# LANL-Bioinformatics/PCRamp

Hardware: AMD Instinct MI355X
Metric: primer-pair x target amplification evals/sec (higher is better)
Workload: dtype u32

## Files before the change

pcramp_amd/csrc/pcr_device.hip:

```cpp
#include <hip/hip_runtime.h>
#include <cstring>
#include <rocprim/device/device_radix_sort.hpp>

#include <stdint.h>
#include <string.h>
#include <math.h>
#include <stdlib.h>
#include <string>
#include <vector>
#include <chrono>
#include <algorithm>
#include <unordered_map>
#include <type_traits>
#include <thread>
#include <mutex>
#include <condition_variable>
#include <functional>
#include <memory>

#include "../../include/pcramp_hip.h"
#include "pcr_host.hpp"

using pcrhost::Planes;

// ... 152 lines not shown
	const uint32_t tagged = (k.epoch << 8) | cnt;
	const uint32_t old = atomicMax(&k.best[(size_t)seq*k.ncand + cand], tagged);
	if(tagged >= old){
		const uint32_t slot = atomicAdd(&k.seq_count[seq], 1u);
		if(slot < k.cap){
			Hit h; h.key = key; h.cand = cand; h.cnt = cnt;
			k.hits[(size_t)seq*k.cap + slot] = h;
		}
		else{ atomicOr(&k.counters[0], 1u); atomicMax(&k.counters[2], slot + 1); }
	}
}

__device__ __noinline__ void record_hit(const HitSink k, uint32_t seq, uint32_t cand, uint64_t key, uint32_t cnt)
{
	record_hit_inline(k, seq, cand, key, cnt);
}

__device__ __forceinline__ uint64_t make_key(uint32_t seq, int32_t loc, uint32_t strand , uint32_t kind, uint32_t ord)
{
	return ((uint64_t)seq << KEY_SEQ_SHIFT) | ((uint64_t)(uint32_t)(loc + LOC_BIAS) << KEY_LOC_SHIFT) |
		((uint64_t)(strand - 1) << 7) | ((uint64_t)kind << 6) | ord;
}

__global__ void k_touched(const uint32_t *__restrict__ seq_count, uint32_t n, uint32_t *__restrict__ counters, uint32_t *__restrict__ touched)
{
	const uint32_t s = blockIdx.x*blockDim.x + threadIdx.x;
	const uint32_t fill = (s < n) ? seq_count[s] : 0u;
	const bool has = fill > 0;
	const uint64_t mask = __ballot(has);
	if(!mask) return;
// ... 426 lines not shown
	pcrhost::PackFilter filt;
	SeqSet sets[PCR_N_SETS];
	DevBuf<uint32_t> best, counters, mask, status;
	int scan_version = 3;
	bool force_seed1 = false;
	std::vector<uint32_t> s2_seeds; std::vector<uint4> s2_masks; std::vector<uint8_t> s2_floors;
	std::vector<uint32_t> s2_group_end, s2_group_offmask, s2_group_or, s2_group_nor;
	struct S2Key { uint32_t a, c, g, t, floor_; bool operator==(const S2Key &o) const { return a == o.a && c == o.c && g == o.g && t == o.t && floor_ == o.floor_; } };
	struct S2KeyHash { size_t operator()(const S2Key &k) const { uint64_t h = 0x9E3779B97F4A7C15ull; for(uint32_t v : {k.a, k.c, k.g, k.t, k.floor_}){ h ^= v; h *= 0x100000001B3ull; h ^= h >> 29; } return (size_t)h; } };
	struct S2Entry { std::vector<uint32_t> seeds;  uint32_t off_mask; bool seedable; uint4 mask;
		std::vector<uint32_t> chunks; uint32_t chunks_total = 0; uint64_t chunks_gen = 0;  };
	std::unordered_map<S2Key, S2Entry, S2KeyHash> s2_cache;
	std::vector<pcrhost::Seed> s2_tmp;
	struct S3Launch { Seed3Slices W; uint32_t n_chunks, per_wg, slice_cap, n_irr_wg; };
	std::vector<S3Launch> s3_launch;
	std::vector<uint32_t> s3_prefix; bool no_seed3 = false, s3_attr_set = false;
	bool s2_attr_set = false; uint32_t s2_dbg = 0; bool no_irr_index = false;
	std::vector<uint32_t> s1_seeds; std::unordered_map<S2Key, S2Entry, S2KeyHash> s1_cache;
	DevBuf<uint32_t> s1_image, s1_heads, s1_multi, s1_part;
	bool host_seed_tables = false;
	DevBuf<Hit> hits;
	DevBuf<uint64_t> bits_fr, bits_rf;
	DevBuf<OligoDev> oligos;
	DevBuf<SwJob> sw_jobs; DevBuf<SwOut> sw_out; DevBuf<uint8_t> sw_q, sw_qlen, sw_t, entry_codes, entry_lens;
	DevBuf<AmpRec> amp_recs, amp_recs2; DevBuf<BgPairDev> bg_pairs;
	DevBuf<uint64_t> amp_keys; DevBuf<uint32_t> amp_pkeys, amp_pair_start; DevBuf<uint8_t> sort_tmp;
	DevBuf<thermo::Job> th_jobs; DevBuf<thermo::JobOut> th_out; DevBuf<int> th_dg; DevBuf<uint2> th_map; DevBuf<uint32_t> th_bad;
	float th_dg_salt = -1.0f;
	DevBuf<unsigned long long> th_dbg; bool th_attr_set = false;
	std::vector<thermo::Job> th_host_jobs; std::vector<thermo::JobOut> th_host_res;
// ... 715 lines not shown
	}
	memset((void *)ctx->mail, 0, sizeof(pcr_ctx::Mail)*pcr_ctx::MAIL_RING);
	return ctx;
}

void pcr_destroy(pcr_ctx *ctx)
{
	if(!ctx) return;
	(void)hipSetDevice(ctx->device);
	(void)hipStreamSynchronize(ctx->stream);
	ctx->pending.clear();
	if(ctx->timing && ctx->n_timed){
		const double n = (double)ctx->n_timed;
		fprintf(stderr, "[pcramp] host us/pass: plan %.1f  stage %.1f  launch %.1f  wait %.1f | amplify prep %.1f  launch %.1f  (%llu passes)\n",
			ctx->t_host[0]/n, ctx->t_host[1]/n, ctx->t_host[2]/n, ctx->t_host[3]/n, ctx->t_host[4]/n, ctx->t_host[5]/n, (unsigned long long)ctx->n_timed);
	}
	for(auto &pr : ctx->prof_events){ (void)hipEventDestroy(pr.first); (void)hipEventDestroy(pr.second); }
	for(int k = 0;k < PCR_PROF_KERNELS;++k){ for(auto &pr : ctx->prof_events_k[k]){ (void)hipEventDestroy(pr.first); (void)hipEventDestroy(pr.second); } }
	for(int s = 0;s < PCR_N_SETS;++s) ctx->sets[s].release();
	ctx->best.release();
	ctx->counters.release(); ctx->mask.release(); ctx->status.release(); ctx->hits.release();
	ctx->s1_image.release(); ctx->s1_heads.release(); ctx->s1_multi.release(); ctx->s1_part.release();
	ctx->bits_fr.release(); ctx->bits_rf.release(); ctx->arena.release(); ctx->fin_scratch.release();
	for(auto &sl : ctx->stage){ if(sl.host) (void)hipHostFree(sl.host); if(sl.done) (void)hipEventDestroy(sl.done); }
	for(auto &sl : ctx->dstage){ if(sl.dev) (void)hipFree(sl.dev); }
	if(ctx->mail) (void)hipHostFree(ctx->mail);
	if(ctx->ret_host) (void)hipHostFree(ctx->ret_host);
	if(ctx->in_host) (void)hipHostFree(ctx->in_host);
	if(ctx->ret_flag) (void)hipHostFree(ctx->ret_flag);
	if(ctx->sw_pin) (void)hipHostFree(ctx->sw_pin);
	for(int k = 0;k < 2;++k){ if(ctx->sw_done[k]) (void)hipEventDestroy(ctx->sw_done[k]); }
// ... 241 lines not shown
	return pcr_split_many(ctx, which, &seq, &pos, 1);
}

}

namespace {

inline uint32_t spread16(uint32_t v)
{
	v &= 0xFFFFu;
	v = (v | (v << 8)) & 0x00FF00FFu; v = (v | (v << 4)) & 0x0F0F0F0Fu;
	v = (v | (v << 2)) & 0x33333333u; return (v | (v << 1)) & 0x55555555u;
}

constexpr uint32_t S2_MAX_GROUPS = 4096;
bool plan_seed2(pcr_ctx *ctx, const std::vector<pcrhost::Candidate> &cand, std::vector<uint32_t> &or_seed, std::vector<uint32_t> &or_plain, uint32_t &irr_off_mask,
	const SeqSet *S3 = nullptr)
{
	std::vector<uint32_t> &pf = ctx->s3_prefix;
	pf.clear();
	uint32_t pf_run = 0;
	const uint32_t n_or = 2*(uint32_t)cand.size();
	std::vector<uint32_t> &out = ctx->s2_seeds;
	out.clear(); ctx->s2_group_end.clear(); ctx->s2_group_offmask.clear(); ctx->s2_group_or.clear(); ctx->s2_group_nor.clear();
	irr_off_mask = 0;
	ctx->s2_masks.resize(n_or);
	if(ctx->s2_cache.size() > 16384) ctx->s2_cache.clear();
	size_t group_begin = 0; uint32_t group_mask = 0, group_or0 = 0, group_last = 0;
	auto fits = [&](size_t n, uint32_t g_or){
		if(S3) return g_or <= S3_MAX_OR && n <= S3_MAX_SEEDS;
		return g_or <= S2_MAX_OR && n <= S2_MAX_SEEDS && sizeof(S2Shared) + 17*(size_t)g_or + 8*n + 1024 <= 160*1024;
	};
	for(uint32_t o = 0;o < n_or;++o){
		const pcrhost::Candidate &c = cand[o >> 1];
		const Planes &m = (o & 1u) ? c.rc : c.fwd;
		const pcr_ctx::S2Key key = {m.a, m.c, m.g, m.t, c.floor_};
		auto it = ctx->s2_cache.find(key);
		if(it == ctx->s2_cache.end()){
			pcr_ctx::S2Entry e; e.off_mask = 0;
			ctx->s2_tmp.clear();
			e.seedable = pcrhost::orientation_seeds(m, c.floor_, 0, ctx->s2_tmp, nullptr, S2_Q);
			e.mask = make_uint4(spread16(m.a) | (spread16(m.a >> 16) << 1), spread16(m.c) | (spread16(m.c >> 16) << 1),
			                    spread16(m.g) | (spread16(m.g >> 16) << 1), spread16(m.t) | (spread16(m.t >> 16) << 1));
			e.seeds.reserve(ctx->s2_tmp.size());
			for(const pcrhost::Seed &sd : ctx->s2_tmp){ e.seeds.push_back((sd.code << 14) | ((uint32_t)sd.off << 9)); e.off_mask |= 1u << sd.off; }
			it = ctx->s2_cache.emplace(key, std::move(e)).first;
		}
		pcr_ctx::S2Entry &e = it->second;
		ctx->s2_masks[o] = e.mask;
		if(!e.seedable){ or_plain.push_back(o); continue; }
		or_seed.push_back(o);
		if(!fits(out.size() - group_begin + e.seeds.size(), o - group_or0 + 1)){
			if(!fits(e.seeds.size(), 1) || ctx->s2_group_end.size() + 1 >= S2_MAX_GROUPS) return false;
			ctx->s2_group_end.push_back((uint32_t)out.size()); ctx->s2_group_offmask.push_back(group_mask); ctx->s2_group_or.push_back(group_or0); ctx->s2_group_nor.push_back(group_last - group_or0 + 1);
			group_begin = out.size(); group_mask = 0; group_or0 = o;
			if(S3){ pf.push_back(pf_run); pf_run = 0; }
		}
		group_last = o;
		const size_t at = out.size();
		out.resize(at + e.seeds.size());
		for(size_t k = 0;k < e.seeds.size();++k) out[at + k] = e.seeds[k] | (o - group_or0);
		if(S3){
			if(e.chunks_gen != S3->pix_generation){
				e.chunks.resize(e.seeds.size());
				uint32_t run = 0;
				for(size_t k = 0;k < e.seeds.size();++k){ e.chunks[k] = run; run += (S3->pix_count_h[e.seeds[k] >> 14] + 63u) >> 6; }
				e.chunks_total = run; e.chunks_gen = S3->pix_generation;
			}
			const size_t pa = pf.size();
			pf.resize(pa + e.chunks.size());
			for(size_t k = 0;k < e.chunks.size();++k) pf[pa + k] = pf_run + e.chunks[k];
			pf_run += e.chunks_total;
		}
		if(!(o & 1u)){ irr_off_mask |= e.off_mask; group_mask |= e.off_mask; }
	}
	ctx->s2_group_end.push_back((uint32_t)out.size()); ctx->s2_group_offmask.push_back(group_mask); ctx->s2_group_or.push_back(group_or0);
	ctx->s2_group_nor.push_back(or_seed.empty() ? 0u : group_last - group_or0 + 1);
	if(S3) pf.push_back(pf_run);
	return true;
}

constexpr size_t S3_LDS_BUDGET = 120*1024;
uint32_t seed3_grid(const pcr_ctx *ctx, int *wg_threads)
{
	static const int s3_wg = getenv("PCRAMP_S3_WG") ? atoi(getenv("PCRAMP_S3_WG")) : 1024;
	static const int s3_per_cu = getenv("PCRAMP_S3_PER_CU") ? atoi(getenv("PCRAMP_S3_PER_CU")) : 0;
	if(wg_threads) *wg_threads = (s3_wg == 1024) ? 1024 : 512;
	return std::min<uint32_t>(ctx->n_cu*(uint32_t)(s3_per_cu ? s3_per_cu : (s3_wg == 1024 ? 2 : 4)), S3_MAX_WG);
}
bool plan_seed3_slices(pcr_ctx *ctx, bool with_irr)
{
	int wg_threads = 0;
	const uint32_t G_all = seed3_grid(ctx, &wg_threads);
	ctx->s3_launch.resize(ctx->s2_group_end.size());
	size_t g_begin = 0, g_prefix = 0;
	for(size_t g = 0;g < ctx->s2_group_end.size();++g){
		const uint32_t ns = ctx->s2_group_end[g] - (uint32_t)g_begin;
		g_begin = ctx->s2_group_end[g];
		const uint32_t *P = ctx->s3_prefix.data() + g_prefix;
		g_prefix += (size_t)ns + 1;
		pcr_ctx::S3Launch &L = ctx->s3_launch[g];
		L.n_irr_wg = with_irr ? std::min<uint32_t>((ns + 16u*(uint32_t)(wg_threads/64) - 1u)/(16u*(uint32_t)(wg_threads/64)), G_all/4u) : 0u;
		const uint32_t G = G_all - L.n_irr_wg;
		L.n_chunks = P[ns]; L.per_wg = std::max<uint32_t>(1u, (L.n_chunks + G - 1u)/G); L.slice_cap = 2;
		if(ns == 0) continue;
		uint32_t at = 0;
		for(uint32_t w = 0;w <= G;++w){
			const uint64_t target = (uint64_t)w*L.per_wg;
			while(at + 1u < ns && P[at + 1u] <= target) ++at;
			L.W.start[w] = at;
		}
		for(uint32_t w = G + 1;w <= S3_MAX_WG;++w) L.W.start[w] = at;
		for(uint32_t w = 0;w < G;++w) L.slice_cap = std::max(L.slice_cap, std::min(L.W.start[w + 1] + 2u, ns + 1u) - L.W.start[w]);
		if(17*(size_t)ctx->s2_group_nor[g] + 8*(size_t)L.slice_cap + 64 > S3_LDS_BUDGET) return false;
	}
	return true;
}

void plan_seed1(pcr_ctx *ctx, const std::vector<pcrhost::Candidate> &cand, std::vector<uint32_t> &or_seed, std::vector<uint32_t> &or_plain, uint32_t &irr_off_mask)
{
	const uint32_t n_or = 2*(uint32_t)cand.size();
	std::vector<uint32_t> &out = ctx->s1_seeds;
	out.clear();
	irr_off_mask = 0;
	if(ctx->s1_cache.size() > 16384) ctx->s1_cache.clear();
// ... 177 lines not shown

int select_impl(pcr_ctx *ctx, pcr_set which, const pcr_pair *pairs, uint32_t n_pairs, int optimize_5, int optimize_3,
	float threshold, uint32_t min_oligo_length, uint64_t *n_entries_out, bool async, FusedAmp *fa = nullptr)
{
	if(!ctx || (n_pairs && !pairs)){ g_err = "pcr_select_words: bad argument"; return PCR_ERR_ARG; }
	if(min_oligo_length < 1 || min_oligo_length > 32){ g_err = "pcr_select_words: min_oligo_length must be in [1,32]"; return PCR_ERR_ARG; }
	HIP_TRY(hipSetDevice(ctx->device));
	SeqSet &S = ctx->sets[which];
	S.have_db = false; S.n_entries = 0;
	if(n_entries_out) *n_entries_out = 0;
	const bool ctrl_was_clean = S.ctrl_clean;
	S.ctrl_clean = false; S.touched_from_seg = false;
	bool lean = false, cleared_bits = false; size_t lean_bits_bytes = 0;
	HostTimer timer(ctx, 0);
	if(ctx->timing) ++ctx->n_timed;
	std::vector<pcrhost::Candidate> cand;
	pcrhost::build_candidates((const uint64_t *)pairs, n_pairs, optimize_5 != 0, optimize_3 != 0, threshold, cand);
	const uint32_t ncand = (uint32_t)cand.size();
	if(S.n == 0 || ncand == 0){ S.have_db = true; S.n_touched = 0; return PCR_OK; }
	std::vector<uint4> hf(ncand), hr(ncand); std::vector<uint32_t> hfl(ncand);
	for(uint32_t c = 0;c < ncand;++c){
		hf[c] = make_uint4(cand[c].fwd.a, cand[c].fwd.c, cand[c].fwd.g, cand[c].fwd.t);
		hr[c] = make_uint4(cand[c].rc.a, cand[c].rc.c, cand[c].rc.g, cand[c].rc.t);
		hfl[c] = cand[c].floor_;
	}
	int rc;
	if((rc = ctx->best.ensure((size_t)S.n*ncand)) != PCR_OK) return rc;
	if(ctx->best.generation != ctx->best_seen){
		HIP_TRY(hipMemsetAsync(ctx->best.p, 0, ctx->best.cap*sizeof(uint32_t), ctx->stream));
		ctx->best_seen = ctx->best.generation; ctx->epoch = std::min(ctx->debug_epoch, EPOCH_LIMIT);
	}
	const uint32_t n_or = 2*ncand;
	std::vector<uint32_t> or_seed, or_plain;
	HostSeedPlan H;
	uint32_t irr_off_mask = 0;
	bool want_seed3 = false, s3_with_irr = false;
	if(ctx->scan_version == 3 && !ctx->force_seed1 && !optimize_5 && !optimize_3 && n_or <= 65535 && !ctx->no_seed3 && !ctx->no_irr_index && ctx->s2_dbg == 0){
		bool worth = true;
		if(!S.pix_valid){
			std::vector<uint32_t> os, op; uint32_t om = 0;
			worth = plan_seed2(ctx, cand, os, op, om, nullptr) && op.empty() && !os.empty();
		}
		if(worth){
			int irc = ensure_pos_index(ctx, S);
			if(irc != PCR_OK) return irc;
			uint32_t n_live0 = 0;
			for(uint32_t k = std::min<uint32_t>(min_oligo_length, 256);k < 256;++k) n_live0 += S.irr_size_count[k];
			bool irr_ok = n_live0 == 0;
			if(S.pix_usable && !irr_ok && S.irr_n_multi == 0 && (uint64_t)24*S.n_irr < (uint64_t(1) << 32)){
				if((irc = ensure_irr_index(ctx, S)) != PCR_OK) return irc;
				irr_ok = S.irx_usable;
			}
			want_seed3 = S.pix_usable && irr_ok; s3_with_irr = n_live0 > 0;
		}
	}
	bool use_seed2 = false;
	if(ctx->scan_version == 3 && !ctx->force_seed1 && !optimize_5 && !optimize_3 && n_or <= 65535){
		use_seed2 = plan_seed2(ctx, cand, or_seed, or_plain, irr_off_mask, want_seed3 ? &S : nullptr);
		if(want_seed3 && !(use_seed2 && or_plain.empty() && !or_seed.empty() && plan_seed3_slices(ctx, s3_with_irr))){
			or_seed.clear(); or_plain.clear();
			use_seed2 = plan_seed2(ctx, cand, or_seed, or_plain, irr_off_mask, nullptr);
		}
		if(use_seed2 && !or_plain.empty() && (n_or <= S1_MAX_OR || or_seed.empty())) use_seed2 = false;
		if(!use_seed2){ or_seed.clear(); or_plain.clear(); irr_off_mask = 0; }
	}
	const bool use_seed3 = use_seed2 && want_seed3 && or_plain.empty() && !or_seed.empty()
		&& ctx->s3_prefix.size() == ctx->s2_seeds.size() + ctx->s2_group_end.size();
	bool dev_tables = false;
	if(!use_seed2 && ctx->scan_version == 3 && !ctx->host_seed_tables && !optimize_5 && !optimize_3 && n_or <= S1_MAX_OR){
		plan_seed1(ctx, cand, or_seed, or_plain, irr_off_mask);
		dev_tables = true;
	}
	if(use_seed2 || dev_tables){  }
	else if(ctx->scan_version == 3 && n_or <= 65535){
// ... 17 lines not shown
	const uint32_t *d_tab_seedset = nullptr, *d_bias_seedset = nullptr, *d_map_seedset = nullptr;
	{
		size_t bytes = ncand*(2*sizeof(uint4) + sizeof(uint32_t)) + 1024;
		bytes += (tab_plain.tab.size() + tab_plain.bias.size() + or_plain.size() + 256)*sizeof(uint32_t);
		bytes += (tab_seedset.tab.size() + tab_seedset.bias.size() + or_seed.size() + 256)*sizeof(uint32_t);
		bytes += (H.image.size() + H.heads.size() + H.multi.size() + 64)*sizeof(uint32_t);
		std::vector<uint4> &masks2 = ctx->s2_masks; std::vector<uint8_t> &floors2 = ctx->s2_floors;
		if(use_seed2){
			floors2.assign(((size_t)n_or + 15) & ~size_t(15), 0);
			for(uint32_t o = 0;o < n_or;++o) floors2[o] = (uint8_t)std::min<uint32_t>(cand[o >> 1].floor_, 255u);
			bytes += masks2.size()*sizeof(uint4) + floors2.size() + ctx->s2_seeds.size()*sizeof(uint32_t) + 512;
			if(use_seed3) bytes += ctx->s3_prefix.size()*sizeof(uint32_t) + 64;
		}
		const bool build_tables = dev_tables && !or_seed.empty();
		if(build_tables) bytes += ctx->s1_seeds.size()*sizeof(uint32_t) + 256;
		std::vector<OligoDev> ol;
		size_t bits_bytes = 0;
		bool fuse = false;
		if(fa && fa->n_pairs){
			bits_bytes = (size_t)fa->n_pairs*((S.n + 63)/64)*sizeof(uint64_t);
			fuse = ((uintptr_t)fa->d_fr % 16 == 0) && ((uintptr_t)fa->d_rf % 16 == 0) && (bits_bytes % 16 == 0);
			if(fuse){ build_oligos(fa->pairs, fa->n_pairs, fa->a, ol); bytes += ol.size()*sizeof(OligoDev) + 64; }
		}
		timer.next(1);
		{
			const uint64_t gen = S.ctrl.generation;
			if((rc = S.ctrl.ensure(8 + 2*(size_t)S.n + 4)) != PCR_OK) return rc;
			lean = ctx->direct_ok && async && fuse && use_seed2 && !or_seed.empty() && ctrl_was_clean && gen == S.ctrl.generation
				&& S.bucket_cap == POST_CAP && 2*fa->n_pairs <= 32*POST_MASK_WORDS;
			lean_bits_bytes = bits_bytes;
		}
// ... 130 lines not shown
						}
						if(use_seed3){
							Seed3Tables T3; T3.seeds = Tg.seeds; T3.chunk_prefix = d_s3_prefix + g_prefix; T3.masks = Tg.masks; T3.floors = Tg.floors;
							g_prefix += Tg.n_seeds + 1u;
							T3.n_seeds = Tg.n_seeds; T3.n_or = Tg.n_or; T3.or_base = Tg.or_base;
							T3.pix_first = S.pix_first.p; T3.pix_last = S.pix_last.p; T3.pix_ent = S.pix_ent.p;
							Seed3Set Q3 = { S.valid_d(), S.blk_info.p, S.blk_local.p, S.d_active.p };
							int s3_wg = 0;
							const uint32_t G = seed3_grid(ctx, &s3_wg);
							const pcr_ctx::S3Launch &L3 = ctx->s3_launch[g];
							T3.n_chunks = L3.n_chunks; T3.per_wg = L3.per_wg; T3.slice_cap = L3.slice_cap;
							T3.n_irr_wg = IA.ix_first ? L3.n_irr_wg : 0u;
							const Seed3Slices &W3 = L3.W;
							const size_t dyn3 = (size_t)g_or*sizeof(uint4) + 2*(size_t)T3.slice_cap*sizeof(uint32_t) + (((size_t)g_or + 15) & ~size_t(15)) + 16;
							if(!ctx->s3_attr_set){
								HIP_TRY(hipFuncSetAttribute((const void *)k_seed3<512>, hipFuncAttributeMaxDynamicSharedMemorySize, 128*1024));
								HIP_TRY(hipFuncSetAttribute((const void *)k_seed3<1024>, hipFuncAttributeMaxDynamicSharedMemorySize, 128*1024));
								ctx->s3_attr_set = true;
							}
							if(s3_wg == 1024) hipLaunchKernelGGL(k_seed3<1024>, dim3(G), dim3(1024), dyn3, ctx->stream, T3, Q3, IA, ctx->d_cand_fwd, ctx->d_cand_floor, sink, Z, W3);
							else hipLaunchKernelGGL(k_seed3<512>, dim3(G), dim3(512), dyn3, ctx->stream, T3, Q3, IA, ctx->d_cand_fwd, ctx->d_cand_floor, sink, Z, W3);
						}
						else if(ctx->s2_dbg)
							hipLaunchKernelGGL(k_seed2<true>, sgrid, sblock, dyn, ctx->stream, S.tb_d(), S.valid_d(), S.tile_desc.p, S.n_tiles, Tg, S.d_active.p, ctx->d_cand_fwd, ctx->d_cand_floor, ncand, IA, sink,
							ctx->s2_dbg, Z);
						else
							hipLaunchKernelGGL(k_seed2<false>, sgrid, sblock, dyn, ctx->stream, S.tb_d(), S.valid_d(), S.tile_desc.p, S.n_tiles, Tg, S.d_active.p, ctx->d_cand_fwd, ctx->d_cand_floor, ncand, IA, sink,
							ctx->s2_dbg, Z);
						HIP_TRY(hipGetLastError());
						first_launch = false;
					}
					if(need_seedset && (rc = launch_scan2(ctx, S, tab_seedset, ncand, sink, d_tab_seedset, d_bias_seedset, S.degen_tiles.p,
						S.n_degen_tiles, d_map_seedset)) != PCR_OK) return rc;
				}
				else if(!or_seed.empty()){
					const bool cand_lds = ncand <= SEED_CAND_LDS;
// ... 458 lines not shown
```

pcramp_amd/csrc/pcr_scan_seed3.inc:

```

constexpr uint32_t PIX_CODES = 1u << 18;
constexpr uint32_t S3_BATCH = 8;

template<bool SCATTER>
__global__ void k_pix_build(const uint32_t *__restrict__ tb, const uint32_t *__restrict__ blk_seq, const uint64_t *__restrict__ blk_off,
	const uint64_t *__restrict__ len, uint64_t total_blocks, uint32_t *__restrict__ count_or_cursor, uint4 *__restrict__ ent)
{
	const uint64_t b = (uint64_t)blockIdx.x*blockDim.x + threadIdx.x;
	if(b >= total_blocks) return;
	const uint32_t seq = blk_seq[b];
	const int64_t p0 = (int64_t)(b - blk_off[seq])*32, L = (int64_t)len[seq];
	uint32_t w[8];
#pragma unroll
	for(int k = 0;k < 8;++k) w[k] = tb[(int64_t)2*(int64_t)b - 2 + k];
#pragma unroll
	for(int i = 0;i < 32;++i){
		if(p0 + i + 9 > L) break;
		const uint32_t code = ((i < 16) ? funnel(w[2], w[3], 2*i) : funnel(w[3], w[4], 2*(i - 16))) & S2_CODE_MASK;
		if(SCATTER){
			const uint32_t at = atomicAdd(&count_or_cursor[code], 1u);
			const int jl = (i + 9) >> 4, sl = 2*((i + 9) & 15);
			const int jr = (i + 41) >> 4, sr = 2*((i + 41) & 15);
			const uint32_t l_lo = funnel(w[jl], w[jl + 1], sl), l_hi = funnel(w[jl + 1], w[jl + 2], sl) & 0x3FFFu;
			const uint32_t r_lo = funnel(w[jr], w[jr + 1], sr), r_hi = funnel(w[jr + 1], w[jr + 2], sr) & 0x3FFFu;
// ... 30 lines not shown
	const uint64_t bl = b - blk_off[q], tile = bl >> 5;
	const uint32_t nt = tile0[q + 1] - tile0[q];
	const bool degen = tile < nt && tile_degen[tile0[q] + tile];
	blk_info[b] = q | (degen ? 0x80000000u : 0u) | (active[q] ? 0u : 0x40000000u);
	blk_local[b] = (uint32_t)bl;
}

__global__ void k_blk_active(uint32_t *__restrict__ blk_info, const uint32_t *__restrict__ blk_seq, const uint8_t *__restrict__ active, uint64_t total_blocks)
{
	const uint64_t b = (uint64_t)blockIdx.x*blockDim.x + threadIdx.x;
	if(b >= total_blocks) return;
	const uint32_t v = blk_info[b] & ~BLK_INACTIVE;
	blk_info[b] = v | (active[blk_seq[b]] ? 0u : BLK_INACTIVE);
}

__device__ __forceinline__ void s3_irregular(const Seed3Tables &T3, const Seed3Set &Q, const IrrArgs2 &IA, const uint4 *__restrict__ cand_fwd,
	const uint32_t *__restrict__ cand_floor, HitSink sink, uint32_t gw, uint32_t n_gw, uint32_t lane)
{
	for(uint32_t i0 = gw*16u;i0 < T3.n_seeds;i0 += n_gw*16u){
		const uint32_t i = i0 + lane;
		const uint32_t sdv = (lane < 16u && i < T3.n_seeds) ? T3.seeds[i] : S2_END;
		const uint32_t orient = T3.or_base + (sdv & 0x1FFu);
		uint32_t first = 0, cnt = 0;
		if(sdv != S2_END && !(orient & 1u)){
			const uint32_t key = (((sdv >> 9) & 31u) << 18) | (sdv >> 14);
			first = IA.ix_first[key]; cnt = IA.ix_last[key] - first;
		}
		const uint32_t incl = s2_scan(cnt);
		const uint32_t total = s2_rl(incl, 63);
		for(uint32_t t0 = 0;t0 < total;t0 += 64u){
			const uint32_t t = t0 + lane;
			uint32_t lo = 0;
#pragma unroll
			for(uint32_t stp = 32u;stp;stp >>= 1){ if((uint32_t)__shfl((int)incl, (int)(lo + stp - 1u)) <= t) lo += stp; }
			const int sl = (int)min(lo, 63u);
			const uint32_t s_incl = (uint32_t)__shfl((int)incl, sl), s_cnt = (uint32_t)__shfl((int)cnt, sl), s_first = (uint32_t)__shfl((int)first, sl);
			const uint32_t c = (uint32_t)__shfl((int)orient, sl) >> 1;
			if(t >= total) continue;
			const IrrDev e = IA.irr[IA.ix_words[s_first + (t - (s_incl - s_cnt))]];
			if(((e.meta >> 8) & 0xFFu) < IA.min_cws || !Q.active[e.seq]) continue;
			const uint32_t n = match_count(e.w.a, e.w.c, e.w.g, e.w.t, cand_fwd[c]);
			if(n >= cand_floor[c]) record_hit(sink, e.seq, c, make_key(e.seq, e.loc, e.meta & 0xFF, 1, (e.meta >> 16) & 0xFF), n);
		}
	}
}

template<uint32_t S3_THREADS>
__global__ __launch_bounds__(S3_THREADS) __attribute__((amdgpu_waves_per_eu(8, 8))) void k_seed3(Seed3Tables T3, Seed3Set Q, IrrArgs2 IA, const uint4 *__restrict__ cand_fwd, const uint32_t *__restrict__ cand_floor,
	HitSink sink, S2Clear Z, Seed3Slices W)
{
	extern __shared__ uint4 s3_dyn[];
	uint4 *const masks = s3_dyn;
	uint32_t *const prefix = (uint32_t *)(masks + T3.n_or);
	uint32_t *const seeds = prefix + T3.slice_cap;
	uint8_t *const floors = (uint8_t *)(seeds + T3.slice_cap);
	const uint32_t wave = threadIdx.x >> 6, lane = threadIdx.x & 63u;
	for(uint32_t i = blockIdx.x*S3_THREADS + threadIdx.x;i < Z.n0;i += gridDim.x*S3_THREADS) Z.z0[i] = make_uint4(0, 0, 0, 0);
	for(uint32_t i = blockIdx.x*S3_THREADS + threadIdx.x;i < Z.n1;i += gridDim.x*S3_THREADS) Z.z1[i] = make_uint4(0, 0, 0, 0);
	if(Z.ctrl && blockIdx.x == 0 && threadIdx.x == 0){ Z.ctrl[1] = 0; Z.ctrl[3] = 0; }
	for(uint32_t i = threadIdx.x;i < T3.n_or;i += S3_THREADS){ masks[i] = T3.masks[i]; floors[i] = T3.floors[i]; }
	constexpr uint32_t S3_WAVES = S3_THREADS/64;
	if(blockIdx.x < T3.n_irr_wg){
		if(IA.ix_first) s3_irregular(T3, Q, IA, cand_fwd, cand_floor, sink, blockIdx.x*S3_WAVES + wave, T3.n_irr_wg*S3_WAVES, lane);
		return;
	}
	const uint32_t wg = blockIdx.x - T3.n_irr_wg, n_wg = gridDim.x - T3.n_irr_wg;
	const uint32_t s_lo = W.start[wg];
	const uint32_t n_slice = min(min(W.start[wg + 1] + 2u, T3.n_seeds + 1u) - s_lo, T3.slice_cap);
	for(uint32_t i = threadIdx.x;i < n_slice;i += S3_THREADS){ prefix[i] = T3.chunk_prefix[s_lo + i]; seeds[i] = (s_lo + i < T3.n_seeds) ? T3.seeds[s_lo + i] : 0u; }
	__syncthreads();
	const uint32_t gw = wg*S3_WAVES + wave, n_gw = n_wg*S3_WAVES;
	const uint32_t q_lo = wg*T3.per_wg, q_hi = min(q_lo + T3.per_wg, T3.n_chunks);
	for(uint32_t q0 = q_lo + wave;q0 < q_hi;q0 += S3_WAVES*S3_BATCH){
		uint32_t c_first = 0, c_cnt = 0, c_sd = 0;
		{
			const uint32_t q = q0 + lane*S3_WAVES;
			if(lane < S3_BATCH && q < q_hi){
				uint32_t lo = 0, hi = n_slice - 1u;
// ... 30 lines not shown
		for(int b = 0;b < (int)S3_BATCH;++b){
			vw[b] = 0; info[b] = 0; bl[b] = 0;
			if(pass_b[b]){
				const uint32_t ws = g[b] - ((s2_rl(c_sd, b) >> 9) & 31u);
				vw[b] = Q.valid[ws >> 5]; info[b] = Q.blk_info[ws >> 5]; bl[b] = Q.blk_local[ws >> 5];
			}
		}
#pragma unroll
		for(int b = 0;b < (int)S3_BATCH;++b){
			if(!pass_b[b]) continue;
			const uint32_t sdv = s2_rl(c_sd, b);
			const uint32_t ws = g[b] - ((sdv >> 9) & 31u), seq = info[b] & BLK_SEQ_MASK;
			if(!((vw[b] >> (ws & 31u)) & 1u) || (info[b] & (BLK_DEGEN | BLK_INACTIVE))) continue;
			const uint32_t p_local = bl[b]*32u + (ws & 31u);
			const uint32_t orient = T3.or_base + (sdv & 0x1FFu), c = orient >> 1;
			if(orient & 1u) record_hit(sink, seq, c, make_key(seq, (int32_t)p_local + 31, 2, 0, 0), cnt_b[b]);
			else record_hit(sink, seq, c, make_key(seq, (int32_t)p_local, 1, 0, 0), cnt_b[b]);
		}
	}
	if(IA.ix_first && T3.n_irr_wg == 0) s3_irregular(T3, Q, IA, cand_fwd, cand_floor, sink, gw, n_gw, lane);
}
```

pcramp_amd/csrc/pcr_screen.inc:

```
__device__ __forceinline__ bool db_slot(uint32_t g, uint32_t n, uint32_t cap, const uint32_t *__restrict__ touched,
	const uint32_t *__restrict__ seg_hi, uint32_t &slot)
{
	if(g >= n) return false;
	const uint32_t seq = touched[g/cap];
	slot = seq*cap + g % cap;
	return slot < seg_hi[seq];
}

constexpr int MATCH_WAVES = 4;
__global__ __launch_bounds__(64*MATCH_WAVES) void k_match(const DevEntry *__restrict__ db, uint32_t n_touched, const uint32_t *__restrict__ n_touched_dev, uint32_t cap,
	const uint32_t *__restrict__ touched, const uint32_t *__restrict__ seg_hi, const OligoDev *__restrict__ oligos, uint32_t n_oligo,
	uint32_t mask_words, uint32_t *__restrict__ mask, uint32_t *__restrict__ status,
	const uint32_t *__restrict__ pub_counters, PassMail *pub_mail, uint32_t pub_seq)
{
	if(blockIdx.x == 0 && threadIdx.x == 0 && status) status[0] = 0;
	if(pub_mail && blockIdx.x == 0 && threadIdx.x < 64){
		if(threadIdx.x < 4) pub_mail->counters[threadIdx.x] = pub_counters[threadIdx.x];
		__threadfence_system();
		__builtin_amdgcn_wave_barrier();
		if(threadIdx.x == 0) __hip_atomic_store((uint32_t *)&pub_mail->seq, pub_seq, __ATOMIC_RELEASE, __HIP_MEMORY_SCOPE_SYSTEM);
	}
	if(n_touched_dev) n_touched = *n_touched_dev;
	const uint32_t lane = threadIdx.x & 63u, sub = lane >> 5, ol = lane & 31u;
	for(uint32_t t_idx = blockIdx.x*MATCH_WAVES + (threadIdx.x >> 6);t_idx < n_touched;t_idx += gridDim.x*MATCH_WAVES){
// ... 262 lines not shown
			const float f = (side == 0) ? var : best, r2 = (side == 0) ? best : var;
			if(__fsqrt_rn(__fmul_rn(f, r2)) >= ident_thr)
				atomicOr((unsigned long long *)&dst[(size_t)v*bit_words + (seq >> 6)], bit);
		}
	}
}

constexpr uint32_t POST_CAP = 64, POST_MASK_WORDS = 4;
struct PostEnt { Planes w; int32_t loc; uint32_t strand; };
template<int POST_WAVES>
struct PostShared {
	OligoDev ol[32*POST_MASK_WORDS];
	uint64_t keys[POST_WAVES][POST_CAP]; PostEnt ent[POST_WAVES][POST_CAP]; uint32_t msk[POST_WAVES][POST_CAP][POST_MASK_WORDS];
};

template<int POST_WAVES>
__global__ __launch_bounds__(64*POST_WAVES) void k_post(const Hit *__restrict__ hits, uint32_t *__restrict__ seq_count,
	const uint32_t *__restrict__ best, uint32_t ncand, const uint4 *__restrict__ planes, const uint64_t *__restrict__ blk_off,
	const IrrDev *__restrict__ irr, const uint32_t *__restrict__ irr_off, DevEntry *__restrict__ db, uint32_t *__restrict__ seg_hi,
	uint32_t *__restrict__ counters, uint32_t epoch, uint32_t n_seq,
	const OligoDev *__restrict__ oligos, uint32_t n_pairs, uint32_t mask_words,
	const uint64_t *__restrict__ len, const uint8_t *__restrict__ active, int32_t amp_min, int32_t amp_max, float ident_thr, int use_taq,
	uint64_t *__restrict__ bits_fr, uint64_t *__restrict__ bits_rf, uint64_t bit_words, PassMail *pub_mail, uint32_t pub_seq)
{
	__shared__ PostShared<POST_WAVES> sh;
	const uint32_t wave = threadIdx.x >> 6, lane = threadIdx.x & 63u;
	if(pub_mail && blockIdx.x == 0 && wave == 0){
		if(lane < 4) pub_mail->counters[lane] = (lane == 3) ? N_TOUCHED_UNKNOWN_DEV : counters[lane];
		__threadfence_system();
		__builtin_amdgcn_wave_barrier();
		if(lane == 0) __hip_atomic_store((uint32_t *)&pub_mail->seq, pub_seq, __ATOMIC_RELEASE, __HIP_MEMORY_SCOPE_SYSTEM);
	}
	if(blockIdx.x == 0 && wave == 0 && lane < 4) counters[lane] = 0;
	const uint32_t seq = blockIdx.x*POST_WAVES + wave;
	const uint32_t n_raw = (seq < n_seq) ? seq_count[seq] : 0u;
	const uint32_t n = min(n_raw, POST_CAP);
	if(seq < n_seq && lane == 0){
		if(n_raw) seq_count[seq] = 0;
		else seg_hi[seq] = 0;
	}
	const uint32_t seq_c = min(seq, n_seq - 1u);
	const uint64_t base = blk_off[seq_c];
	const int32_t L = (int32_t)len[seq_c];
	const uint32_t is_active = active[seq_c];
	if(__syncthreads_or((int)n)){
		const uint32_t nw = 2*n_pairs*(uint32_t)(sizeof(OligoDev)/4);
		for(uint32_t i = threadIdx.x;i < nw;i += 64*POST_WAVES) ((uint32_t *)sh.ol)[i] = ((const uint32_t *)oligos)[i];
		__syncthreads();
	}
	if(n == 0) return;
	uint64_t *keys = sh.keys[wave];
	PostEnt *ent = sh.ent[wave];
	uint64_t k = ~0ull;
	if(lane < n){
		const Hit h = hits[(size_t)seq*POST_CAP + lane];
		if(((epoch << 8) | h.cnt) == best[(size_t)seq*ncand + h.cand]) k = h.key;
	}
	keys[lane] = k;
	wave_sync();
	uint32_t np2 = 1; while(np2 < n) np2 <<= 1;
	for(uint32_t kk = 2;kk <= np2;kk <<= 1){
		for(uint32_t j = kk >> 1;j > 0;j >>= 1){
			const uint32_t l = lane ^ j;
			if(l > lane && l < np2){
				const uint64_t a = keys[lane], b = keys[l];
				const bool up = ((lane & kk) == 0);
				if((a > b) == up){ keys[lane] = b; keys[l] = a; }
			}
			wave_sync();
		}
	}
	k = keys[lane];
// ... 215 lines not shown
```

Before: 19.76 billion.

## Append seed3 hits without atomicMax and resolve per-candidate best in k_post

Adds an APPEND variant of k_seed3 that writes hits straight into the per-sequence list, skipping the global atomicMax on the best table. k_post now computes each candidate's maximum count itself by scanning the wave's hits in LDS. The variant is used in lean mode. On the host, the seed3 workgroup slice boundaries are computed during the plan_seed2 prefix walk rather than in a second pass, and per-pass vectors are reused from the context. Without the atomicMax filter, more hits may reach the per-sequence cap and overflow. The k_post scan is O(n) per lane over at most 64 entries.

After: 20.53 billion (median of 6 runs). 1.04x the previous value.

```diff
diff --git a/pcramp_amd/csrc/pcr_device.hip b/pcramp_amd/csrc/pcr_device.hip
--- a/pcramp_amd/csrc/pcr_device.hip
+++ b/pcramp_amd/csrc/pcr_device.hip
@@ -190,6 +190,23 @@
 __device__ __noinline__ void record_hit(const HitSink k, uint32_t seq, uint32_t cand, uint64_t key, uint32_t cnt)
 {
 	record_hit_inline(k, seq, cand, key, cnt);
+}
+
+__device__ __noinline__ void append_hit(const HitSink k, uint32_t seq, uint32_t cand, uint64_t key, uint32_t cnt)
+{
+	const uint32_t slot = atomicAdd(&k.seq_count[seq], 1u);
+	if(slot < k.cap){
+		Hit h; h.key = key; h.cand = cand; h.cnt = cnt;
+		k.hits[(size_t)seq*k.cap + slot] = h;
+	}
+	else{ atomicOr(&k.counters[0], 1u); atomicMax(&k.counters[2], slot + 1); }
+}
+
+template<bool APPEND>
+__device__ __forceinline__ void sink_hit(const HitSink &k, uint32_t seq, uint32_t cand, uint64_t key, uint32_t cnt)
+{
+	if(APPEND) append_hit(k, seq, cand, key, cnt);
+	else record_hit(k, seq, cand, key, cnt);
 }
 
 __device__ __forceinline__ uint64_t make_key(uint32_t seq, int32_t loc, uint32_t strand , uint32_t kind, uint32_t ord)
@@ -646,6 +663,9 @@
 	std::vector<pcrhost::Seed> s2_tmp;
 	struct S3Launch { Seed3Slices W; uint32_t n_chunks, per_wg, slice_cap, n_irr_wg; };
 	std::vector<S3Launch> s3_launch;
+	std::vector<S2Entry *> s2_ent;
+	bool s3_walked = false; uint32_t s3_walk_G = 0, s3_walk_per_wg = 0;
+	std::vector<pcrhost::Candidate> pass_cand; std::vector<uint4> pass_hf, pass_hr; std::vector<uint32_t> pass_hfl; std::vector<OligoDev> pass_ol;
 	std::vector<uint32_t> s3_prefix; bool no_seed3 = false, s3_attr_set = false;
 	bool s2_attr_set = false; uint32_t s2_dbg = 0; bool no_irr_index = false;
 	std::vector<uint32_t> s1_seeds; std::unordered_map<S2Key, S2Entry, S2KeyHash> s1_cache;
@@ -1391,7 +1411,19 @@
 		const double n = (double)ctx->n_timed;
 		fprintf(stderr, "[pcramp] host us/pass: plan %.1f  stage %.1f  launch %.1f  wait %.1f | amplify prep %.1f  launch %.1f  (%llu passes)\n",
 			ctx->t_host[0]/n, ctx->t_host[1]/n, ctx->t_host[2]/n, ctx->t_host[3]/n, ctx->t_host[4]/n, ctx->t_host[5]/n, (unsigned long long)ctx->n_timed);
-	}
+		fprintf(stderr, "[pcramp] host: of the plan, workgroup slices %.1f us/pass; index builds (once per set, not in the plan) %.1f ms\n",
+			ctx->t_host[7]/n, ctx->t_host[6]*1e-3);
+	}
+#ifdef PCRAMP_FILL_HIST
+	{
+		uint32_t h[257];
+		if(hipMemcpyFromSymbol(h, HIP_SYMBOL(g_fill_hist), sizeof(h)) == hipSuccess){
+			fprintf(stderr, "[pcramp] bucket fills offered to k_post (fill:sequence-passes):");
+			for(int i = 0;i < 257;++i) if(h[i]) fprintf(stderr, " %d:%u", i, h[i]);
+			fprintf(stderr, "\n");
+		}
+	}
+#endif
 	for(auto &pr : ctx->prof_events){ (void)hipEventDestroy(pr.first); (void)hipEventDestroy(pr.second); }
 	for(int k = 0;k < PCR_PROF_KERNELS;++k){ for(auto &pr : ctx->prof_events_k[k]){ (void)hipEventDestroy(pr.first); (void)hipEventDestroy(pr.second); } }
 	for(int s = 0;s < PCR_N_SETS;++s) ctx->sets[s].release();
@@ -1663,9 +1695,12 @@
 }
 
 constexpr uint32_t S2_MAX_GROUPS = 4096;
+uint32_t seed3_grid(const pcr_ctx *ctx, int *wg_threads);
+uint32_t s3_irr_wgs(uint32_t ns, int wg_threads, uint32_t G_all, bool with_irr);
 bool plan_seed2(pcr_ctx *ctx, const std::vector<pcrhost::Candidate> &cand, std::vector<uint32_t> &or_seed, std::vector<uint32_t> &or_plain, uint32_t &irr_off_mask,
-	const SeqSet *S3 = nullptr)
-{
+	const SeqSet *S3 = nullptr, bool s3_with_irr = false)
+{
+	ctx->s3_walked = false;
 	std::vector<uint32_t> &pf = ctx->s3_prefix;
 	pf.clear();
 	uint32_t pf_run = 0;
@@ -1680,6 +1715,9 @@
 		if(S3) return g_or <= S3_MAX_OR && n <= S3_MAX_SEEDS;
 		return g_or <= S2_MAX_OR && n <= S2_MAX_SEEDS && sizeof(S2Shared) + 17*(size_t)g_or + 8*n + 1024 <= 160*1024;
 	};
+	std::vector<pcr_ctx::S2Entry *> &ent = ctx->s2_ent;
+	ent.resize(n_or);
+	size_t tot_seeds = 0; uint64_t tot_chunks = 0; uint32_t o_first = n_or, o_last = 0;
 	for(uint32_t o = 0;o < n_or;++o){
 		const pcrhost::Candidate &c = cand[o >> 1];
 		const Planes &m = (o & 1u) ? c.rc : c.fwd;
@@ -1696,6 +1734,30 @@
 			it = ctx->s2_cache.emplace(key, std::move(e)).first;
 		}
 		pcr_ctx::S2Entry &e = it->second;
+		ent[o] = &e;
+		if(!e.seedable) continue;
+		if(S3 && e.chunks_gen != S3->pix_generation){
+			e.chunks.resize(e.seeds.size());
+			uint32_t run = 0;
+			for(size_t k = 0;k < e.seeds.size();++k){ e.chunks[k] = run; run += (S3->pix_count_h[e.seeds[k] >> 14] + 63u) >> 6; }
+			e.chunks_total = run; e.chunks_gen = S3->pix_generation;
+		}
+		tot_seeds += e.seeds.size(); tot_chunks += S3 ? e.chunks_total : 0u;
+		o_first = std::min(o_first, o); o_last = o;
+	}
+	pcr_ctx::S3Launch *WL = nullptr;
+	uint32_t w_next = 0, w_G = 0, w_per = 0; uint64_t w_target = 0;
+	if(S3 && tot_seeds && fits(tot_seeds, o_last - o_first + 1) && tot_chunks < (uint64_t(1) << 32)){
+		int wg_threads = 0;
+		const uint32_t G_all = seed3_grid(ctx, &wg_threads);
+		w_G = G_all - s3_irr_wgs((uint32_t)tot_seeds, wg_threads, G_all, s3_with_irr);
+		w_per = std::max<uint32_t>(1u, (uint32_t)((tot_chunks + w_G - 1u)/w_G));
+		ctx->s3_launch.resize(1);
+		WL = &ctx->s3_launch[0];
+		WL->W.start[0] = 0; w_next = 1; w_target = w_per;
+	}
+	for(uint32_t o = 0;o < n_or;++o){
+		pcr_ctx::S2Entry &e = *ent[o];
 		ctx->s2_masks[o] = e.mask;
 		if(!e.seedable){ or_plain.push_back(o); continue; }
 		or_seed.push_back(o);
@@ -1710,15 +1772,13 @@
 		out.resize(at + e.seeds.size());
 		for(size_t k = 0;k < e.seeds.size();++k) out[at + k] = e.seeds[k] | (o - group_or0);
 		if(S3){
-			if(e.chunks_gen != S3->pix_generation){
-				e.chunks.resize(e.seeds.size());
-				uint32_t run = 0;
-				for(size_t k = 0;k < e.seeds.size();++k){ e.chunks[k] = run; run += (S3->pix_count_h[e.seeds[k] >> 14] + 63u) >> 6; }
-				e.chunks_total = run; e.chunks_gen = S3->pix_generation;
-			}
 			const size_t pa = pf.size();
 			pf.resize(pa + e.chunks.size());
-			for(size_t k = 0;k < e.chunks.size();++k) pf[pa + k] = pf_run + e.chunks[k];
+			for(size_t k = 0;k < e.chunks.size();++k){
+				const uint32_t v = pf_run + e.chunks[k];
+				pf[pa + k] = v;
+				while(WL && w_next <= w_G && (uint64_t)v > w_target){ WL->W.start[w_next] = (uint32_t)(pa + k) - 1u; ++w_next; w_target += w_per; }
+			}
 			pf_run += e.chunks_total;
 		}
 		if(!(o & 1u)){ irr_off_mask |= e.off_mask; group_mask |= e.off_mask; }
@@ -1726,10 +1786,19 @@
 	ctx->s2_group_end.push_back((uint32_t)out.size()); ctx->s2_group_offmask.push_back(group_mask); ctx->s2_group_or.push_back(group_or0);
 	ctx->s2_group_nor.push_back(or_seed.empty() ? 0u : group_last - group_or0 + 1);
 	if(S3) pf.push_back(pf_run);
+	if(WL){
+		for(;w_next <= w_G;++w_next) WL->W.start[w_next] = (uint32_t)tot_seeds - 1u;
+		ctx->s3_walked = true; ctx->s3_walk_G = w_G; ctx->s3_walk_per_wg = w_per;
+	}
 	return true;
 }
 
 constexpr size_t S3_LDS_BUDGET = 120*1024;
+uint32_t s3_irr_wgs(uint32_t ns, int wg_threads, uint32_t G_all, bool with_irr)
+{
+	const uint32_t per_wg = 16u*(uint32_t)(wg_threads/64);
+	return with_irr ? std::min<uint32_t>((ns + per_wg - 1u)/per_wg, G_all/4u) : 0u;
+}
 uint32_t seed3_grid(const pcr_ctx *ctx, int *wg_threads)
 {
 	static const int s3_wg = getenv("PCRAMP_S3_WG") ? atoi(getenv("PCRAMP_S3_WG")) : 1024;
@@ -1749,15 +1818,18 @@
 		const uint32_t *P = ctx->s3_prefix.data() + g_prefix;
 		g_prefix += (size_t)ns + 1;
 		pcr_ctx::S3Launch &L = ctx->s3_launch[g];
-		L.n_irr_wg = with_irr ? std::min<uint32_t>((ns + 16u*(uint32_t)(wg_threads/64) - 1u)/(16u*(uint32_t)(wg_threads/64)), G_all/4u) : 0u;
+		L.n_irr_wg = s3_irr_wgs(ns, wg_threads, G_all, with_irr);
 		const uint32_t G = G_all - L.n_irr_wg;
 		L.n_chunks = P[ns]; L.per_wg = std::max<uint32_t>(1u, (L.n_chunks + G - 1u)/G); L.slice_cap = 2;
 		if(ns == 0) continue;
-		uint32_t at = 0;
-		for(uint32_t w = 0;w <= G;++w){
-			const uint64_t target = (uint64_t)w*L.per_wg;
-			while(at + 1u < ns && P[at + 1u] <= target) ++at;
-			L.W.start[w] = at;
+		uint32_t at = ns - 1u;
+		if(!(ctx->s3_walked && ctx->s2_group_end.size() == 1 && ctx->s3_walk_G == G && ctx->s3_walk_per_wg == L.per_wg)){
+			at = 0;
+			for(uint32_t w = 0;w <= G;++w){
+				const uint64_t target = (uint64_t)w*L.per_wg;
+				while(at + 1u < ns && P[at + 1u] <= target) ++at;
+				L.W.start[w] = at;
+			}
 		}
 		for(uint32_t w = G + 1;w <= S3_MAX_WG;++w) L.W.start[w] = at;
 		for(uint32_t w = 0;w < G;++w) L.slice_cap = std::max(L.slice_cap, std::min(L.W.start[w + 1] + 2u, ns + 1u) - L.W.start[w]);
@@ -1965,11 +2037,13 @@
 	bool lean = false, cleared_bits = false; size_t lean_bits_bytes = 0;
 	HostTimer timer(ctx, 0);
 	if(ctx->timing) ++ctx->n_timed;
-	std::vector<pcrhost::Candidate> cand;
+	std::vector<pcrhost::Candidate> &cand = ctx->pass_cand;
+	cand.clear();
 	pcrhost::build_candidates((const uint64_t *)pairs, n_pairs, optimize_5 != 0, optimize_3 != 0, threshold, cand);
 	const uint32_t ncand = (uint32_t)cand.size();
 	if(S.n == 0 || ncand == 0){ S.have_db = true; S.n_touched = 0; return PCR_OK; }
-	std::vector<uint4> hf(ncand), hr(ncand); std::vector<uint32_t> hfl(ncand);
+	std::vector<uint4> &hf = ctx->pass_hf, &hr = ctx->pass_hr; std::vector<uint32_t> &hfl = ctx->pass_hfl;
+	hf.resize(ncand); hr.resize(ncand); hfl.resize(ncand);
 	for(uint32_t c = 0;c < ncand;++c){
 		hf[c] = make_uint4(cand[c].fwd.a, cand[c].fwd.c, cand[c].fwd.g, cand[c].fwd.t);
 		hr[c] = make_uint4(cand[c].rc.a, cand[c].rc.c, cand[c].rc.g, cand[c].rc.t);
@@ -1993,6 +2067,7 @@
 			worth = plan_seed2(ctx, cand, os, op, om, nullptr) && op.empty() && !os.empty();
 		}
 		if(worth){
+			timer.next(6);
 			int irc = ensure_pos_index(ctx, S);
 			if(irc != PCR_OK) return irc;
 			uint32_t n_live0 = 0;
@@ -2003,12 +2078,16 @@
 				irr_ok = S.irx_usable;
 			}
 			want_seed3 = S.pix_usable && irr_ok; s3_with_irr = n_live0 > 0;
+			timer.next(0);
 		}
 	}
 	bool use_seed2 = false;
 	if(ctx->scan_version == 3 && !ctx->force_seed1 && !optimize_5 && !optimize_3 && n_or <= 65535){
-		use_seed2 = plan_seed2(ctx, cand, or_seed, or_plain, irr_off_mask, want_seed3 ? &S : nullptr);
-		if(want_seed3 && !(use_seed2 && or_plain.empty() && !or_seed.empty() && plan_seed3_slices(ctx, s3_with_irr))){
+		use_seed2 = plan_seed2(ctx, cand, or_seed, or_plain, irr_off_mask, want_seed3 ? &S : nullptr, s3_with_irr);
+		timer.next(7);
+		const bool s3_planned = want_seed3 && use_seed2 && or_plain.empty() && !or_seed.empty() && plan_seed3_slices(ctx, s3_with_irr);
+		timer.next(0);
+		if(want_seed3 && !s3_planned){
 			or_seed.clear(); or_plain.clear();
 			use_seed2 = plan_seed2(ctx, cand, or_seed, or_plain, irr_off_mask, nullptr);
 		}
@@ -2056,7 +2135,8 @@
 		}
 		const bool build_tables = dev_tables && !or_seed.empty();
 		if(build_tables) bytes += ctx->s1_seeds.size()*sizeof(uint32_t) + 256;
-		std::vector<OligoDev> ol;
+		std::vector<OligoDev> &ol = ctx->pass_ol;
+		ol.clear();
 		size_t bits_bytes = 0;
 		bool fuse = false;
 		if(fa && fa->n_pairs){
@@ -2217,12 +2297,16 @@
 							const Seed3Slices &W3 = L3.W;
 							const size_t dyn3 = (size_t)g_or*sizeof(uint4) + 2*(size_t)T3.slice_cap*sizeof(uint32_t) + (((size_t)g_or + 15) & ~size_t(15)) + 16;
 							if(!ctx->s3_attr_set){
-								HIP_TRY(hipFuncSetAttribute((const void *)k_seed3<512>, hipFuncAttributeMaxDynamicSharedMemorySize, 128*1024));
-								HIP_TRY(hipFuncSetAttribute((const void *)k_seed3<1024>, hipFuncAttributeMaxDynamicSharedMemorySize, 128*1024));
+								HIP_TRY(hipFuncSetAttribute((const void *)k_seed3<512, false>, hipFuncAttributeMaxDynamicSharedMemorySize, 128*1024));
+								HIP_TRY(hipFuncSetAttribute((const void *)k_seed3<1024, false>, hipFuncAttributeMaxDynamicSharedMemorySize, 128*1024));
+								HIP_TRY(hipFuncSetAttribute((const void *)k_seed3<512, true>, hipFuncAttributeMaxDynamicSharedMemorySize, 128*1024));
+								HIP_TRY(hipFuncSetAttribute((const void *)k_seed3<1024, true>, hipFuncAttributeMaxDynamicSharedMemorySize, 128*1024));
 								ctx->s3_attr_set = true;
 							}
-							if(s3_wg == 1024) hipLaunchKernelGGL(k_seed3<1024>, dim3(G), dim3(1024), dyn3, ctx->stream, T3, Q3, IA, ctx->d_cand_fwd, ctx->d_cand_floor, sink, Z, W3);
-							else hipLaunchKernelGGL(k_seed3<512>, dim3(G), dim3(512), dyn3, ctx->stream, T3, Q3, IA, ctx->d_cand_fwd, ctx->d_cand_floor, sink, Z, W3);
+#define S3_ARGS dim3(G), dim3(s3_wg == 1024 ? 1024 : 512), dyn3, ctx->stream, T3, Q3, IA, ctx->d_cand_fwd, ctx->d_cand_floor, sink, Z, W3
+							if(lean) hipLaunchKernelGGL((s3_wg == 1024 ? k_seed3<1024, true> : k_seed3<512, true>), S3_ARGS);
+							else hipLaunchKernelGGL((s3_wg == 1024 ? k_seed3<1024, false> : k_seed3<512, false>), S3_ARGS);
+#undef S3_ARGS
 						}
 						else if(ctx->s2_dbg)
 							hipLaunchKernelGGL(k_seed2<true>, sgrid, sblock, dyn, ctx->stream, S.tb_d(), S.valid_d(), S.tile_desc.p, S.n_tiles, Tg, S.d_active.p, ctx->d_cand_fwd, ctx->d_cand_floor, ncand, IA, sink,
diff --git a/pcramp_amd/csrc/pcr_scan_seed3.inc b/pcramp_amd/csrc/pcr_scan_seed3.inc
--- a/pcramp_amd/csrc/pcr_scan_seed3.inc
+++ b/pcramp_amd/csrc/pcr_scan_seed3.inc
@@ -68,6 +68,7 @@
 	blk_info[b] = v | (active[blk_seq[b]] ? 0u : BLK_INACTIVE);
 }
 
+template<bool APPEND>
 __device__ __forceinline__ void s3_irregular(const Seed3Tables &T3, const Seed3Set &Q, const IrrArgs2 &IA, const uint4 *__restrict__ cand_fwd,
 	const uint32_t *__restrict__ cand_floor, HitSink sink, uint32_t gw, uint32_t n_gw, uint32_t lane)
 {
@@ -94,12 +95,12 @@
 			const IrrDev e = IA.irr[IA.ix_words[s_first + (t - (s_incl - s_cnt))]];
 			if(((e.meta >> 8) & 0xFFu) < IA.min_cws || !Q.active[e.seq]) continue;
 			const uint32_t n = match_count(e.w.a, e.w.c, e.w.g, e.w.t, cand_fwd[c]);
-			if(n >= cand_floor[c]) record_hit(sink, e.seq, c, make_key(e.seq, e.loc, e.meta & 0xFF, 1, (e.meta >> 16) & 0xFF), n);
+			if(n >= cand_floor[c]) sink_hit<APPEND>(sink, e.seq, c, make_key(e.seq, e.loc, e.meta & 0xFF, 1, (e.meta >> 16) & 0xFF), n);
 		}
 	}
 }
 
-template<uint32_t S3_THREADS>
+template<uint32_t S3_THREADS, bool APPEND>
 __global__ __launch_bounds__(S3_THREADS) __attribute__((amdgpu_waves_per_eu(8, 8))) void k_seed3(Seed3Tables T3, Seed3Set Q, IrrArgs2 IA, const uint4 *__restrict__ cand_fwd, const uint32_t *__restrict__ cand_floor,
 	HitSink sink, S2Clear Z, Seed3Slices W)
 {
@@ -115,7 +116,7 @@
 	for(uint32_t i = threadIdx.x;i < T3.n_or;i += S3_THREADS){ masks[i] = T3.masks[i]; floors[i] = T3.floors[i]; }
 	constexpr uint32_t S3_WAVES = S3_THREADS/64;
 	if(blockIdx.x < T3.n_irr_wg){
-		if(IA.ix_first) s3_irregular(T3, Q, IA, cand_fwd, cand_floor, sink, blockIdx.x*S3_WAVES + wave, T3.n_irr_wg*S3_WAVES, lane);
+		if(IA.ix_first) s3_irregular<APPEND>(T3, Q, IA, cand_fwd, cand_floor, sink, blockIdx.x*S3_WAVES + wave, T3.n_irr_wg*S3_WAVES, lane);
 		return;
 	}
 	const uint32_t wg = blockIdx.x - T3.n_irr_wg, n_wg = gridDim.x - T3.n_irr_wg;
@@ -176,9 +177,9 @@
 			if(!((vw[b] >> (ws & 31u)) & 1u) || (info[b] & (BLK_DEGEN | BLK_INACTIVE))) continue;
 			const uint32_t p_local = bl[b]*32u + (ws & 31u);
 			const uint32_t orient = T3.or_base + (sdv & 0x1FFu), c = orient >> 1;
-			if(orient & 1u) record_hit(sink, seq, c, make_key(seq, (int32_t)p_local + 31, 2, 0, 0), cnt_b[b]);
-			else record_hit(sink, seq, c, make_key(seq, (int32_t)p_local, 1, 0, 0), cnt_b[b]);
+			if(orient & 1u) sink_hit<APPEND>(sink, seq, c, make_key(seq, (int32_t)p_local + 31, 2, 0, 0), cnt_b[b]);
+			else sink_hit<APPEND>(sink, seq, c, make_key(seq, (int32_t)p_local, 1, 0, 0), cnt_b[b]);
 		}
 	}
-	if(IA.ix_first && T3.n_irr_wg == 0) s3_irregular(T3, Q, IA, cand_fwd, cand_floor, sink, gw, n_gw, lane);
+	if(IA.ix_first && T3.n_irr_wg == 0) s3_irregular<APPEND>(T3, Q, IA, cand_fwd, cand_floor, sink, gw, n_gw, lane);
 }
diff --git a/pcramp_amd/csrc/pcr_screen.inc b/pcramp_amd/csrc/pcr_screen.inc
--- a/pcramp_amd/csrc/pcr_screen.inc
+++ b/pcramp_amd/csrc/pcr_screen.inc
@@ -300,6 +300,9 @@
 	uint64_t keys[POST_WAVES][POST_CAP]; PostEnt ent[POST_WAVES][POST_CAP]; uint32_t msk[POST_WAVES][POST_CAP][POST_MASK_WORDS];
 };
 
+#ifdef PCRAMP_FILL_HIST
+__device__ uint32_t g_fill_hist[257];
+#endif
 template<int POST_WAVES>
 __global__ __launch_bounds__(64*POST_WAVES) void k_post(const Hit *__restrict__ hits, uint32_t *__restrict__ seq_count,
 	const uint32_t *__restrict__ best, uint32_t ncand, const uint4 *__restrict__ planes, const uint64_t *__restrict__ blk_off,
@@ -319,13 +322,18 @@
 	}
 	if(blockIdx.x == 0 && wave == 0 && lane < 4) counters[lane] = 0;
 	const uint32_t seq = blockIdx.x*POST_WAVES + wave;
+	const uint32_t seq_c = min(seq, n_seq - 1u);
 	const uint32_t n_raw = (seq < n_seq) ? seq_count[seq] : 0u;
 	const uint32_t n = min(n_raw, POST_CAP);
+	Hit h; h.key = 0; h.cand = 0; h.cnt = 0;
+	if(lane < n) h = hits[(size_t)seq*POST_CAP + lane];
+#ifdef PCRAMP_FILL_HIST
+	if(seq < n_seq && lane == 0) atomicAdd(&g_fill_hist[min(n_raw, 256u)], 1u);
+#endif
 	if(seq < n_seq && lane == 0){
 		if(n_raw) seq_count[seq] = 0;
 		else seg_hi[seq] = 0;
 	}
-	const uint32_t seq_c = min(seq, n_seq - 1u);
 	const uint64_t base = blk_off[seq_c];
 	const int32_t L = (int32_t)len[seq_c];
 	const uint32_t is_active = active[seq_c];
@@ -337,11 +345,14 @@
 	if(n == 0) return;
 	uint64_t *keys = sh.keys[wave];
 	PostEnt *ent = sh.ent[wave];
-	uint64_t k = ~0ull;
-	if(lane < n){
-		const Hit h = hits[(size_t)seq*POST_CAP + lane];
-		if(((epoch << 8) | h.cnt) == best[(size_t)seq*ncand + h.cand]) k = h.key;
-	}
+	uint32_t *tags = (uint32_t *)keys;
+	const uint32_t tag = (lane < n) ? ((h.cand << 8) | h.cnt) : 0xFFFFFFFFu;
+	tags[lane] = tag;
+	wave_sync();
+	uint32_t mx = 0;
+	for(uint32_t j = 0;j < n;++j){ const uint32_t t = tags[j]; if((t >> 8) == (tag >> 8)) mx = max(mx, t & 0xFFu); }
+	wave_sync();
+	uint64_t k = (lane < n && (tag & 0xFFu) == mx) ? h.key : ~0ull;
 	keys[lane] = k;
 	wave_sync();
 	uint32_t np2 = 1; while(np2 < n) np2 <<= 1;
```
